# TUMFTM/RadarGNN

Hardware: AMD Instinct MI355X
Metric: radar frames/sec (graph-build + GNN fwd) (higher is better)
Workload: dtype f32 (dense layers: fp32 operands split into 2 f16 terms after an exact power-of-two pre-scale, 3 f16 MFMA products per fp32 product, fp32 accumulate -- more accurate than fp32 MFMA against float64, tests/test_gpu_f16x2.py; RGNN_NO_F16X2=1 selects 3 bf16 terms / 6 products, RGNN_LINEAR_FP32=1 v_mfma_; 1 GPU; C2: per GPU 64 RadarScenes-shaped frames x 3000 pts, radius graph r=1.0, node feats [rcs,velocity_vector,time_index,degree], edge feats [relative_position], 4-layer MPNNConv [224,224,128,64] + emb MLPs + both heads, train-mode BatchNorm, max aggr; frames_per_gpu=64, points_per_gpu=192000, edges_per_gpu=799078, ranks_in_process_group=1

## Files before the change

### include/rgnn.h

```cpp
#ifndef RGNN_H
#define RGNN_H

#include <stdint.h>

#ifdef __cplusplus
extern "C" {
#endif

typedef void* rgnn_stream_t;

#define RGNN_OK 0
#define RGNN_ERR_INVALID_ARGUMENT (-1)
#define RGNN_ERR_LAUNCH (-2)
#define RGNN_ERR_UNSUPPORTED (-3)

#define RGNN_STATUS_KNN_TOO_FEW_POINTS 1
#define RGNN_STATUS_DOT_PRODUCT 2
#define RGNN_STATUS_TIME_INDEX_OVERFLOW 4
#define RGNN_STATUS_EDGE_COUNT_CHANGED 8
#define RGNN_STATUS_NOT_SYMMETRIC 16
#define RGNN_STATUS_SPLITK_TIMEOUT 32
#define RGNN_STATUS_GT_OBJECT_TOO_LARGE 64
#define RGNN_STATUS_GT_DEGENERATE_OBJECT 128
#define RGNN_STATUS_PREPROCESS_BAD_ROW 256
// ... 214 lines not shown
                                const float* in_bound, float* out_bound, rgnn_stream_t stream);
int rgnn_batchnorm_segments_from_panels(const float* stats_a, const int32_t* panel_start_a, const float* stats_b,
                                        const int32_t* panel_start_b, const int64_t* seg_ptr, int64_t n_seg, int32_t n,
                                        const float* gamma, const float* beta, float* running_mean, float* running_var,
                                        int64_t* num_batches_tracked, float momentum, float eps, double* seg_sums, float* table,
                                        const float* in_bound, float* out_bound, rgnn_stream_t stream);
int rgnn_pad_list_by_segment(const int32_t* list, const int64_t* count, const int64_t* seg_ptr, int64_t n_seg, int32_t* out_list,
                             int64_t* out_count, int32_t* tile_segment, int32_t* stat_panel_start, rgnn_stream_t stream);
int rgnn_pad_list_pair_by_segment(const int32_t* list_a, const int64_t* count_a, const int32_t* list_b, const int64_t* count_b,
                                  const int64_t* seg_ptr, int64_t n_seg, int32_t* out_list_a, int64_t* out_count_a,
                                  int32_t* tile_segment_a, int32_t* stat_panel_start_a, int32_t* out_list_b, int64_t* out_count_b,
                                  int32_t* tile_segment_b, int32_t* stat_panel_start_b, rgnn_stream_t stream);
int rgnn_scale_shift_act_segments(const float* x, int64_t ldx, const float* table, const int64_t* seg_ptr, int64_t n_seg,
                                  int64_t m, int32_t n, int32_t relu, float* y, int64_t ldy, rgnn_stream_t stream);
int rgnn_column_stats(const float* x, int64_t ldx, int64_t m, int32_t n, float* col_stats ,
                      rgnn_stream_t stream);
int rgnn_scale_shift_act(const float* x, int64_t ldx, const float* scale_shift, int64_t m, int32_t n, int32_t relu,
                         float* y, int64_t ldy, rgnn_stream_t stream);

#define RGNN_AGGR_MAX 0
#define RGNN_AGGR_MEAN 1
#define RGNN_AGGR_ADD 2
int rgnn_mpnn_aggregate(const float* P, int64_t ldp, const float* p_bias, const float* Q, int64_t ldq,
                        const float* We , int64_t ldwe, const float* edge_attr_sorted,
                        int32_t de, const int32_t* rowptr_t, const int32_t* src_sorted,
                        const int32_t* node_order ,
                        const int32_t* chunk_start , int32_t n_chunks, int64_t n,
                        int32_t d, int32_t aggr, float* out, int64_t ldo, rgnn_stream_t stream);

#define RGNN_MPNN_SKIP_EMPTY_ROWS 1
int rgnn_mpnn_aggregate_flags(const float* P, int64_t ldp, const float* p_bias, const float* Q, int64_t ldq,
                              const float* We, int64_t ldwe, const float* edge_attr_sorted, int32_t de,
                              const int32_t* rowptr_t, const int32_t* src_sorted, const int32_t* node_order,
                              const int32_t* chunk_start, int32_t n_chunks, int64_t n, int32_t d, int32_t aggr, float* out,
                              int64_t ldo, int32_t flags, rgnn_stream_t stream);
int rgnn_mpnn_aggregate_absmax(const float* P, int64_t ldp, const float* p_bias, const float* Q, int64_t ldq,
                               const float* We, int64_t ldwe, const float* edge_attr_sorted, int32_t de,
                               const int32_t* rowptr_t, const int32_t* src_sorted, const int32_t* node_order,
                               const int32_t* chunk_start, int32_t n_chunks, int64_t n, int32_t d, int32_t aggr, float* out,
                               int64_t ldo, int32_t flags, float* out_absmax, rgnn_stream_t stream);
int rgnn_mpnn_aggregate_max_arg(const float* p_bias, const float* Q, int64_t ldq, const float* We, int64_t ldwe,
                                const float* edge_attr_sorted, int32_t de, const int32_t* rowptr_t, const int32_t* src_sorted,
                                const int32_t* node_order, const int32_t* chunk_start, int32_t n_chunks, int64_t n, int32_t d,
                                float* out, int64_t ldo, uint16_t* arg_out, int32_t flags, int32_t* arg_written ,
                                rgnn_stream_t stream);
int rgnn_mpnn_aggregate_max_arg_absmax(const float* p_bias, const float* Q, int64_t ldq, const float* We, int64_t ldwe,
                                       const float* edge_attr_sorted, int32_t de, const int32_t* rowptr_t, const int32_t* src_sorted,
                                       const int32_t* node_order, const int32_t* chunk_start, int32_t n_chunks, int64_t n, int32_t d,
                                       float* out, int64_t ldo, uint16_t* arg_out, int32_t flags, int32_t* arg_written ,
                                       float* out_absmax, rgnn_stream_t stream);

int64_t rgnn_mpnn_win_plan_ints(int64_t n, int64_t n_edges);
void rgnn_mpnn_win_plan_counters(int64_t n, int64_t n_edges, int64_t* leftover_word , int64_t* windows_word );
int rgnn_mpnn_win_plan(const int32_t* rowptr_t, const int32_t* src_sorted, const int32_t* node_order, int64_t n, int64_t n_edges,
                       int32_t* plan, rgnn_stream_t stream);
int rgnn_mpnn_aggregate_win(const float* p_bias, const float* Q, int64_t ldq, const float* We, int64_t ldwe,
                            const float* edge_attr_sorted, int32_t de, const int32_t* rowptr_t, const int32_t* src_sorted,
                            const int32_t* node_order, int32_t* plan, int64_t n, int64_t n_edges, int32_t d, float* out, int64_t ldo,
                            int32_t flags, float* out_absmax, rgnn_stream_t stream);
int64_t rgnn_mpnn_win_wplanes_bytes(int32_t d);
int rgnn_mpnn_win_wplanes(const float* We, int64_t ldwe, int32_t de, int32_t d, const float* p_bias, void* planes, rgnn_stream_t stream);
int rgnn_mpnn_aggregate_win_planes(const float* p_bias, const float* Q, int64_t ldq, const float* We, int64_t ldwe,
                                   const float* edge_attr_sorted, int32_t de, const int32_t* rowptr_t, const int32_t* src_sorted,
                                   const int32_t* node_order, int32_t* plan, int64_t n, int64_t n_edges, int32_t d, float* out,
                                   int64_t ldo, int32_t flags, float* out_absmax, const void* wplanes, rgnn_stream_t stream);

int rgnn_empty_targets(const int32_t* rowptr_t, const int32_t* node_order, int64_t n, int32_t* flags_tmp,
                       int32_t* pos_tmp, void* scan_tmp, int32_t* list, int64_t* count,
                       int32_t* slot_of_node ,
                       rgnn_stream_t stream);

int rgnn_split_targets(const int32_t* rowptr_t, const int32_t* node_order, int64_t n, int32_t* flags_tmp, int32_t* pos_tmp,
                       void* scan_tmp, int32_t* list, int64_t* count, int32_t* slot_of_node, int32_t* list_nonempty,
                       int64_t* count_nonempty, rgnn_stream_t stream);

int rgnn_split_targets_by_node(const int32_t* rowptr_t, const int32_t* rank, int64_t n, int32_t* flags_tmp, int32_t* pos_tmp,
                               void* scan_tmp, int32_t* list, int64_t* count, int32_t* slot_of_node,
                               int32_t* list_nonempty, int64_t* count_nonempty, rgnn_stream_t stream);

int32_t rgnn_mpnn_num_chunks(int64_t n, int64_t n_edges);
int32_t rgnn_mpnn_work_units(int64_t n, int64_t n_edges);
int32_t rgnn_mpnn_target_weight(int64_t n, int64_t n_edges);
int rgnn_mpnn_partition(const int32_t* rowptr_t, int64_t n, int64_t n_edges, int32_t* chunk_start, rgnn_stream_t stream);

int rgnn_mpnn_edge_hidden(const float* P, int64_t ldp, const float* p_bias, const float* Q, int64_t ldq,
                          const float* We, int64_t ldwe, const float* edge_attr_sorted, int32_t de,
                          const int32_t* rowptr_t, const int32_t* src_sorted, const int32_t* node_order,
                          const int32_t* chunk_start, int32_t n_chunks, int64_t n, int32_t d, int32_t relu, float* hidden,
                          int64_t ldh, rgnn_stream_t stream);
int rgnn_segment_reduce(const float* rows, int64_t ldr, const int32_t* rowptr_t, const int32_t* node_order, int64_t n,
                        int32_t d, int32_t aggr, float* out, int64_t ldo, rgnn_stream_t stream);

int rgnn_gather_rows_f32(const float* in, int64_t ldi, const int32_t* perm, int64_t n_rows, int32_t width, float* out,
                         int64_t ldo, rgnn_stream_t stream);

int rgnn_softmax_rows(const float* x, int64_t ldx, int64_t m, int32_t n, float* y, int64_t ldy, rgnn_stream_t stream);

int rgnn_collate_rows(const void* src, int64_t ld_src, int32_t width, const int64_t* seg_src_row, const int64_t* seg_dst_ptr,
                      int32_t n_seg, int64_t n_rows, void* out, int64_t ld_out, int64_t* batch_out, rgnn_stream_t stream);
int rgnn_collate_edges(const int64_t* src_edge_index, int64_t ld_src, const int64_t* seg_src_edge,
                       const int64_t* seg_dst_eptr, const int64_t* seg_node_shift, int32_t n_seg, int64_t n_edges,
                       int64_t* out, int64_t ld_out, rgnn_stream_t stream);

int rgnn_stage_frames(int64_t n_frames, const void* const* addr, const int64_t* n_points, void* block, int64_t block_bytes);

int rgnn_decode_predictions(const float* class_prob, int64_t ldp, int32_t n_classes, const float* boxes, int64_t ldb,
// ... 139 lines not shown
```

### radargnn_amd/_lib.py

```python
from __future__ import annotations

import ctypes as C
import os

import torch

_HERE = os.path.dirname(os.path.abspath(__file__))
LIB_PATH = os.environ.get("RGNN_LIB") or os.path.join(_HERE, "librgnn.so")

c_i32, c_i64, c_f32, c_f64, c_vp = C.c_int32, C.c_int64, C.c_float, C.c_double, C.c_void_p


class RgnnGrid(C.Structure):
    _fields_ = [("X", c_vp), ("dim", c_i32), ("n", c_i64), ("frame_ptr", c_vp), ("n_frames", c_i64),
                ("ws", c_vp), ("ws_bytes", c_i64)]


class RgnnLinearArgs(C.Structure):
    _fields_ = [("A1", c_vp), ("lda1", c_i64), ("k1", c_i32),
                ("A2", c_vp), ("lda2", c_i64), ("k2", c_i32),
                ("W1", c_vp), ("W2", c_vp), ("ldw", c_i64), ("w_split", c_i32),
                ("bias1", c_vp), ("bias2", c_vp),
                ("residual", c_vp), ("ldr", c_i64),
                ("out", c_vp), ("ldo", c_i64),
# ... 46 lines not shown
                            c_vp, c_vp]),
    "rgnn_csr_by_target_symmetric_own": (c_i32, [c_vp, c_vp, c_i64, c_i64, c_vp, c_vp, c_vp, c_vp, c_vp, c_vp, c_vp]),
    "rgnn_edge_features": (c_i32, [c_vp, c_vp, c_vp, c_i64, C.POINTER(c_i32), c_i32, c_i32, c_vp, c_i32, c_vp, c_vp]),
    "rgnn_edge_features_reversed": (c_i32, [c_vp, c_vp, c_vp, c_i64, c_vp, c_i64, C.POINTER(c_i32), c_i32, c_i32, c_vp, c_i32, c_vp, c_vp]),
    "rgnn_node_features": (c_i32, [c_vp, c_vp, c_vp, c_vp, c_vp, c_i64, C.POINTER(c_i32), c_i32, c_vp, c_i32, c_vp]),
    "rgnn_node_features_time_index": (c_i32, [c_vp, c_vp, c_vp, c_vp, c_vp, c_i64, c_vp, c_i64, C.POINTER(c_i32), c_i32, c_vp, c_i32,
                                              c_vp, c_vp, c_vp]),
    "rgnn_split_by_degree_frames": (c_i32, [c_vp, c_vp, c_i64, c_vp, c_vp, c_vp, c_vp, c_vp, c_vp, c_vp]),
    "rgnn_radius_counts": (c_i32, [c_vp, c_i64, c_vp, c_i32, c_vp, c_vp]),
    "rgnn_time_index": (c_i32, [c_vp, c_vp, c_i64, c_vp, c_vp, c_vp]),
    "rgnn_time_index_ws_bytes": (c_i64, [c_i64]),
    "rgnn_time_index_ws": (c_i32, [c_vp, c_vp, c_i64, c_i64, c_vp, c_vp, c_vp, c_i64, c_vp]),
    "rgnn_linear_stat_panels": (c_i64, [c_i64]),
    "rgnn_linear_fwd": (c_i32, [C.POINTER(RgnnLinearArgs), c_vp]),
    "rgnn_linear_fwd_fuses_a1_affine": (c_i32, [C.POINTER(RgnnLinearArgs)]),
    "rgnn_linear_fwd_plan": (None, [C.POINTER(RgnnLinearArgs), C.POINTER(c_i32 * 8)]),
    "rgnn_linear_planes_kp": (c_i32, [c_i32]),
    "rgnn_linear_fwd_path": (c_i32, [C.POINTER(RgnnLinearArgs)]),
    "rgnn_linear_planes_f16_bytes": (c_i64, [c_i32, c_i32]),
    "rgnn_linear_split_weights_f16": (c_i32, [c_vp, c_vp, c_i64, c_i32, c_i32, c_i32, c_vp, c_vp]),
    "rgnn_linear_splitk_ws_bytes": (c_i64, []),
    "rgnn_linear_split_weights": (c_i32, [c_vp, c_vp, c_i64, c_i32, c_i32, c_i32, c_vp, c_vp]),
    "rgnn_tiny_mlp2": (c_i32, [c_vp, c_i64, c_i32, c_vp, c_i64, c_vp, c_i64, c_vp, c_i32, c_i32, c_vp, c_i64, c_vp, c_i32, c_i32, c_vp,
                       c_i64, c_vp]),
    "rgnn_batchnorm_finalize": (c_i32, [c_vp, c_i64, c_i64, c_i32, c_vp, c_vp, c_vp, c_vp, c_vp, c_i32, c_f32, c_f32,
                                        c_vp, c_vp]),
    "rgnn_batchnorm_finalize_parts": (c_i32, [c_vp, c_i64, c_vp, c_vp, c_i64, c_vp, c_i64, c_i32, c_vp, c_vp, c_vp, c_vp, c_vp, c_i32,
                                              c_f32, c_f32, c_vp, c_vp]),
    "rgnn_batchnorm_finalize_bound": (c_i32, [c_vp, c_i64, c_vp, c_vp, c_i64, c_vp, c_i64, c_i32, c_vp, c_vp, c_vp, c_vp, c_vp, c_i32,
                                              c_f32, c_f32, c_vp, c_vp, c_vp, c_vp]),
    "rgnn_batchnorm_segments": (c_i32, [c_vp, c_i64, c_vp, c_i64, c_i32, c_vp, c_vp, c_vp, c_vp, c_vp, c_f32, c_f32, c_vp, c_vp,
                                        c_vp, c_vp, c_vp]),
    "rgnn_batchnorm_act_segments": (c_i32, [c_vp, c_i64, c_vp, c_i64, c_i32, c_vp, c_vp, c_vp, c_vp, c_vp, c_f32, c_f32, c_i32, c_vp,
                                            c_vp, c_vp, c_i64, c_vp, c_vp, c_vp]),
    "rgnn_batchnorm_segments_from_panels": (c_i32, [c_vp, c_vp, c_vp, c_vp, c_vp, c_i64, c_i32, c_vp, c_vp, c_vp, c_vp, c_vp, c_f32,
                                                    c_f32, c_vp, c_vp, c_vp, c_vp, c_vp]),
    "rgnn_pad_list_by_segment": (c_i32, [c_vp, c_vp, c_vp, c_i64, c_vp, c_vp, c_vp, c_vp, c_vp]),
    "rgnn_pad_list_pair_by_segment": (c_i32, [c_vp, c_vp, c_vp, c_vp, c_vp, c_i64, c_vp, c_vp, c_vp, c_vp, c_vp, c_vp, c_vp, c_vp, c_vp]),
    "rgnn_scale_shift_act_segments": (c_i32, [c_vp, c_i64, c_vp, c_vp, c_i64, c_i64, c_i32, c_i32, c_vp, c_i64, c_vp]),
    "rgnn_column_stats": (c_i32, [c_vp, c_i64, c_i64, c_i32, c_vp, c_vp]),
    "rgnn_scale_shift_act": (c_i32, [c_vp, c_i64, c_vp, c_i64, c_i32, c_i32, c_vp, c_i64, c_vp]),
    "rgnn_mpnn_aggregate": (c_i32, [c_vp, c_i64, c_vp, c_vp, c_i64, c_vp, c_i64, c_vp, c_i32, c_vp, c_vp, c_vp, c_vp, c_i32,
                                    c_i64, c_i32, c_i32, c_vp, c_i64, c_vp]),
    "rgnn_mpnn_aggregate_flags": (c_i32, [c_vp, c_i64, c_vp, c_vp, c_i64, c_vp, c_i64, c_vp, c_i32, c_vp, c_vp, c_vp, c_vp, c_i32,
                                          c_i64, c_i32, c_i32, c_vp, c_i64, c_i32, c_vp]),
    "rgnn_mpnn_aggregate_absmax": (c_i32, [c_vp, c_i64, c_vp, c_vp, c_i64, c_vp, c_i64, c_vp, c_i32, c_vp, c_vp, c_vp, c_vp, c_i32,
                                           c_i64, c_i32, c_i32, c_vp, c_i64, c_i32, c_vp, c_vp]),
    "rgnn_mpnn_aggregate_max_arg": (c_i32, [c_vp, c_vp, c_i64, c_vp, c_i64, c_vp, c_i32, c_vp, c_vp, c_vp, c_vp, c_i32, c_i64, c_i32,
                                             c_vp, c_i64, c_vp, c_i32, C.POINTER(c_i32), c_vp]),
    "rgnn_mpnn_aggregate_max_arg_absmax": (c_i32, [c_vp, c_vp, c_i64, c_vp, c_i64, c_vp, c_i32, c_vp, c_vp, c_vp, c_vp, c_i32, c_i64, c_i32,
                                                    c_vp, c_i64, c_vp, c_i32, C.POINTER(c_i32), c_vp, c_vp]),
    "rgnn_mpnn_win_plan_ints": (c_i64, [c_i64, c_i64]),
    "rgnn_mpnn_win_plan_counters": (None, [c_i64, c_i64, C.POINTER(c_i64), C.POINTER(c_i64)]),
    "rgnn_mpnn_win_plan": (c_i32, [c_vp, c_vp, c_vp, c_i64, c_i64, c_vp, c_vp]),
    "rgnn_mpnn_aggregate_win": (c_i32, [c_vp, c_vp, c_i64, c_vp, c_i64, c_vp, c_i32, c_vp, c_vp, c_vp, c_vp, c_i64, c_i64, c_i32, c_vp,
                                        c_i64, c_i32, c_vp, c_vp]),
    "rgnn_mpnn_win_wplanes_bytes": (c_i64, [c_i32]),
    "rgnn_mpnn_win_wplanes": (c_i32, [c_vp, c_i64, c_i32, c_i32, c_vp, c_vp, c_vp]),
    "rgnn_mpnn_aggregate_win_planes": (c_i32, [c_vp, c_vp, c_i64, c_vp, c_i64, c_vp, c_i32, c_vp, c_vp, c_vp, c_vp, c_i64, c_i64, c_i32, c_vp,
                                               c_i64, c_i32, c_vp, c_vp, c_vp]),
    "rgnn_empty_targets": (c_i32, [c_vp, c_vp, c_i64, c_vp, c_vp, c_vp, c_vp, c_vp, c_vp, c_vp]),
    "rgnn_split_targets": (c_i32, [c_vp, c_vp, c_i64, c_vp, c_vp, c_vp, c_vp, c_vp, c_vp, c_vp, c_vp, c_vp]),
    "rgnn_split_targets_by_node": (c_i32, [c_vp, c_vp, c_i64, c_vp, c_vp, c_vp, c_vp, c_vp, c_vp, c_vp, c_vp, c_vp]),
    "rgnn_mpnn_num_chunks": (c_i32, [c_i64, c_i64]),
    "rgnn_mpnn_work_units": (c_i32, [c_i64, c_i64]),
    "rgnn_mpnn_target_weight": (c_i32, [c_i64, c_i64]),
    "rgnn_mpnn_partition": (c_i32, [c_vp, c_i64, c_i64, c_vp, c_vp]),
    "rgnn_mpnn_edge_hidden": (c_i32, [c_vp, c_i64, c_vp, c_vp, c_i64, c_vp, c_i64, c_vp, c_i32, c_vp, c_vp, c_vp, c_vp, c_i32,
                                      c_i64, c_i32, c_i32, c_vp, c_i64, c_vp]),
    "rgnn_segment_reduce": (c_i32, [c_vp, c_i64, c_vp, c_vp, c_i64, c_i32, c_i32, c_vp, c_i64, c_vp]),
    "rgnn_gather_rows_f32": (c_i32, [c_vp, c_i64, c_vp, c_i64, c_i32, c_vp, c_i64, c_vp]),
    "rgnn_softmax_rows": (c_i32, [c_vp, c_i64, c_i64, c_i32, c_vp, c_i64, c_vp]),
    "rgnn_relu_bwd": (c_i32, [c_vp, c_vp, c_vp, c_i64, c_vp]),
    "rgnn_bn_bwd_stats": (c_i32, [c_vp, c_i64, c_vp, c_i64, c_vp, c_i64, c_i64, c_i32, c_vp, c_vp]),
    "rgnn_bn_bwd_apply": (c_i32, [c_vp, c_i64, c_vp, c_i64, c_vp, c_i64, c_vp, c_i64, c_i32, c_vp, c_i64, c_vp]),
    "rgnn_bn_bwd_stats_table": (c_i32, [c_vp, c_i64, c_vp, c_i64, c_vp, c_vp, c_i64, c_i64, c_i32, c_vp, c_vp]),
    "rgnn_bn_bwd_apply_table": (c_i32, [c_vp, c_i64, c_vp, c_i64, c_vp, c_vp, c_i64, c_vp, c_i64, c_i32, c_vp, c_i64, c_vp, c_vp]),
    "rgnn_bn_bwd_apply_absmax": (c_i32, [c_vp, c_i64, c_vp, c_i64, c_vp, c_i64, c_vp, c_i64, c_i32, c_vp, c_i64, c_vp, c_vp]),
    "rgnn_bn_bwd_coef": (c_i32, [c_vp, c_i64, c_vp, c_vp, c_vp, c_i64, c_i64, c_i32, c_vp, c_f32, c_i32, c_vp, c_vp, c_vp, c_vp]),
    "rgnn_mpnn_aggregate_bwd": (c_i32, [c_vp, c_i64, c_vp, c_i64, c_vp, c_i64, c_vp, c_i32, c_vp, c_vp, c_vp, c_i64, c_i32,
                                        c_i32, c_vp, c_vp, c_vp, c_vp, c_i64, c_vp, c_vp, c_vp, c_vp, c_i64, c_vp, c_vp, c_vp]),
    "rgnn_mpnn_max_bwd_supported": (c_i32, [c_i32, c_i32]),
    "rgnn_mpnn_max_bwd": (c_i32, [c_vp, c_i64, c_vp, c_i64, c_vp, c_i64, c_vp, c_i32, c_vp, c_vp, c_vp, c_vp, c_vp, c_i64, c_i32, c_vp,
                                   c_vp, c_vp, c_i64, c_vp, c_i32, c_vp, c_vp, c_i64, c_vp, c_vp, c_vp]),
    "rgnn_mpnn_max_bwd_absmax": (c_i32, [c_vp, c_i64, c_vp, c_i64, c_vp, c_i64, c_vp, c_i32, c_vp, c_vp, c_vp, c_vp, c_vp, c_i64, c_i32, c_vp,
                                          c_vp, c_vp, c_i64, c_vp, c_i32, c_vp, c_vp, c_i64, c_vp, c_vp, c_vp, c_vp]),
    "rgnn_mpnn_bwd_split": (c_i32, [c_i32]),
    "rgnn_segment_reduce_bwd": (c_i32, [c_vp, c_i64, c_vp, c_i64, c_vp, c_vp, c_i64, c_i32, c_i32, c_vp, c_i64, c_vp]),
    "rgnn_linear_wgrad_slabs": (c_i32, [c_i64, c_i32, c_i32]),
    "rgnn_linear_wgrad": (c_i32, [c_vp, c_i64, c_vp, c_i64, c_i32, c_vp, c_i64, c_i32, c_i64, c_i32, c_vp, c_vp, c_vp]),
    "rgnn_wgrad_slabs": (c_i32, [c_i64, c_i32, c_i32, c_i32, c_i32]),
    "rgnn_wgrad": (c_i32, [c_vp, c_i64, c_i32, c_vp, c_i64, c_i32, c_vp, c_i64, c_i32, c_i32, c_i64, c_vp, c_vp, c_vp, c_vp, c_vp]),
    "rgnn_wgrad_bounds": (c_i32, [c_vp, c_i64, c_i32, c_vp, c_i64, c_i32, c_vp, c_i64, c_i32, c_i32, c_i64, c_vp, c_vp, c_vp, c_vp, c_vp, c_vp,
                                   c_vp, c_vp]),
    "rgnn_mpnn_bwd_slots": (c_i64, [c_i64]),
    "rgnn_decode_predictions": (c_i32, [c_vp, c_i64, c_i32, c_vp, c_i64, c_i32, c_vp, c_vp, c_i64, c_i32, C.c_float, c_vp, c_i32,
                                        c_i32, c_i32, c_vp, c_vp, c_vp, c_vp, c_vp]),
    "rgnn_box_representations": (c_i32, [c_vp, c_i64, c_vp, c_vp, c_vp]),
    "rgnn_sort_scores_tmp_bytes": (c_i64, [c_i64]),
    "rgnn_sort_scores": (c_i32, [c_vp, c_i32, c_i64, c_vp, c_vp, c_vp]),
    "rgnn_nms_mask_words": (c_i64, [c_i64]),
    "rgnn_nms": (c_i32, [c_vp, c_i32, c_vp, c_i64, c_f64, c_vp, c_vp, c_vp, c_vp]),
    "rgnn_decode_ground_truth": (c_i32, [c_vp, c_i64, c_vp, c_i64, c_i32, c_vp, c_vp, c_i64, c_i32, c_i32, c_vp, c_vp, c_vp]),
    "rgnn_remove_duplicate_boxes": (c_i32, [c_vp, c_vp, c_i64, c_i64, c_vp, c_vp]),
    "rgnn_point_iou_tmp_bytes": (c_i64, [c_i64, c_i32, c_i64, c_i64]),
    "rgnn_point_iou": (c_i32, [c_vp, c_vp, c_i64, c_vp, c_vp, c_i64, c_i32, c_vp, c_vp, c_i64, c_i32, c_vp, c_i64, c_vp, c_vp, c_vp]),
# ... 55 lines not shown
```

### radargnn_amd/csrc/mpnn_tiles.hip

```cpp
#include "common.h"
#include <stdlib.h>
#include <type_traits>

namespace {

constexpr int MT_THREADS = 256;
constexpr int MT_WAVES = MT_THREADS / 64;
constexpr int MT_QUEUE_INTS = 8 * 16;

typedef float mt_f32x16 __attribute__((ext_vector_type(16)));
typedef __bf16 mt_bf16x8 __attribute__((ext_vector_type(8)));
typedef unsigned int mt_u32x4 __attribute__((ext_vector_type(4)));

__global__ __launch_bounds__(256) void k_tiles_zero_empty(const int32_t* __restrict__ rowptr, const int32_t* __restrict__ order,
                                                         int64_t n, int d, float* __restrict__ out, int64_t ldo) {
  const int lane = threadIdx.x & 63;
  const int64_t p = (int64_t)blockIdx.x * MT_WAVES + (threadIdx.x >> 6);
  if (p >= n || rowptr[p + 1] != rowptr[p]) return;
  const int64_t node = order ? order[p] : p;
  for (int c = lane; c < d; c += 64) out[node * ldo + c] = 0.f;
}

__device__ __forceinline__ void mt_split3(float x, unsigned& t1, unsigned& t2, unsigned& t3) {
  t1 = __float_as_uint(x) & 0xffff0000u;
// ... 262 lines not shown
#pragma unroll
          for (int i = 0; i < 16; i++) c[i] = *(const __attribute__((address_space(3))) float*)(uintptr_t)(unsigned)(aoff[t][i] + ST * WN_ROWBUF);
          c = __builtin_amdgcn_mfma_f32_32x32x16_bf16(__builtin_bit_cast(mt_bf16x8, a3[t]), __builtin_bit_cast(mt_bf16x8, byc), c, 0, 0, 0);
          c = __builtin_amdgcn_mfma_f32_32x32x16_bf16(__builtin_bit_cast(mt_bf16x8, a2[t]), __builtin_bit_cast(mt_bf16x8, bxc), c, 0, 0, 0);
          c = __builtin_amdgcn_mfma_f32_32x32x16_bf16(__builtin_bit_cast(mt_bf16x8, a1[t]), __builtin_bit_cast(mt_bf16x8, bxc), c, 0, 0, 0);
#pragma unroll
          for (int g = 0; g < WN_GPT; g++) {
            rn = __builtin_fmaxf(__builtin_fmaxf(rn, c[WN_PAD * g]), c[WN_PAD * g + 1]);
            if (WN_PAD == 4) rn = __builtin_fmaxf(__builtin_fmaxf(rn, c[WN_PAD * g + 2]), c[WN_PAD * g + 3]);
            if ((anyend >> (WN_GPT * t + g)) & 1u) {
              const int k = WN_GPT * t + g;
              const float v = rn + biasc;
              const unsigned long long mA = ((endA >> k) & 1u) ? 0xffffffffull : 0ull, mB = ((endB >> k) & 1u) ? 0xffffffff00000000ull : 0ull;
              const int soA = __builtin_amdgcn_readlane(tv, k) + ct * 128, soB = __builtin_amdgcn_readlane(tv, 32 + k) + ct * 128;
              if (!(p.abl & 4)) {
                const int off = (half ? soB : soA) + voffc;
                asm volatile("s_mov_b64 exec, %3\n\tbuffer_store_dword %0, %1, %2, 0 offen nt\n\ts_mov_b64 exec, -1"
                             : : "v"(v), "v"(off), "s"(ro_l), "s"(mA | mB) : "memory");
              }
              if (AMAX) amax = fmaxf(amax, fabsf(v));
              const unsigned long long m64 = mA | mB;
              asm volatile("v_cndmask_b32_e64 %0, %0, %1, %2" : "+v"(rn) : "v"(ninf_l), "s"(m64));
            }
          }
        }
      }
    };
    float amax_full = 0.f;
    for (int ct = 0; ct < p.n_ct; ct++) {
      const bool partial = AMAX && (ct + 1) * 32 > p.d;
      if (partial) { amax_full = amax; amax = 0.f; }
      if ((gp + ct) & 1) tile_pass(ct, std::integral_constant<int, 1>());
      else tile_pass(ct, std::integral_constant<int, 0>());
      if (partial) amax = fmaxf(amax_full, (ct * 32 + col < p.d) ? amax : 0.f);
    }
    if (p.n_ct < 2) {
      asm volatile("s_waitcnt vmcnt(0)" ::: "memory");
      __syncthreads();
    }
    gp = (gp + p.n_ct) & 1;
    win = nxt; up ^= 1; staged = staged_next;
  }
  if (AMAX) {
#pragma unroll
    for (int o = 32; o > 0; o >>= 1) amax = fmaxf(amax, __shfl_xor(amax, o, 64));
    if (lane == 0)
      atomicMax((unsigned int*)p.out_absmax + ((blockIdx.x * 4 + wave) & (RGNN_BOUND_SLOTS - 1)), __float_as_uint(amax));
  }
}

constexpr int WN_BIG = 64;

constexpr int WN_SEG = 512;
struct WinPlanLayout {
  int n_win, n_seg;
  int64_t off_assign, off_segcnt, off_segbase, off_wend, off_pdeg, off_wstart, off_left, off_leftcnt, off_queue, off_misc, off_tgt, off_eid, off_lrow, off_urow,
      off_wplanes, total_ints;
};
WinPlanLayout win_layout(int64_t n, int64_t n_edges) {
  WinPlanLayout L;
  L.n_seg = (int)((n + WN_SEG - 1) / WN_SEG);
  L.n_win = (int)((n_edges + 3 * n) / 256 + L.n_seg + 2);
  int64_t o = 16;
  auto take = [&](int64_t ints) { const int64_t at = o; o = (o + ints + 15) / 16 * 16; return at; };
  L.off_assign = take(n + 1); L.off_segcnt = take(L.n_seg + 1); L.off_segbase = take(L.n_seg + 2);
  L.off_wend = take(L.n_win + 1);
  L.off_pdeg = take(n + 1); L.off_wstart = take(L.n_win + 1); L.off_left = take(n + 1); L.off_leftcnt = take(4);
  L.off_queue = take(MT_QUEUE_INTS); L.off_misc = take(16 * (int64_t)L.n_win);
  L.off_tgt = take(8 * WN_GPS * (int64_t)L.n_win); L.off_eid = take(512 * (int64_t)L.n_win); L.off_lrow = take(128 * (int64_t)L.n_win);
  L.off_urow = take(WN_UMAX * (int64_t)L.n_win); L.off_wplanes = take(16 * 64 * 32);
  L.total_ints = o;
  return L;
}

__global__ __launch_bounds__(256) void k_win_pdeg(const int32_t* __restrict__ rowptr, int64_t n, int32_t* __restrict__ pdeg,
                                                 int32_t* __restrict__ left, int32_t* __restrict__ leftcnt, int32_t* __restrict__ queue) {
  const int64_t p = (int64_t)blockIdx.x * blockDim.x + threadIdx.x;
  if (p < MT_QUEUE_INTS) queue[p] = 0;
  if (p > n) return;
  if (p == n) { pdeg[p] = 0; return; }
  const int d = rowptr[p + 1] - rowptr[p];
  const int pd = (d + WN_PAD - 1) & ~(WN_PAD - 1);
  if (pd > WN_BIG) left[atomicAdd(leftcnt, 1)] = (int32_t)p;
  pdeg[p] = (pd > WN_BIG) ? 0 : pd;
}
__global__ __launch_bounds__(64) void k_win_greedy(const int32_t* __restrict__ pdeg, int64_t n, int32_t* __restrict__ assign,
                                                  int32_t* __restrict__ segcnt) {
  __shared__ int spd[WN_SEG];
  __shared__ int sas[WN_SEG];
  const int seg = blockIdx.x, lane = threadIdx.x;
  const int64_t p0 = (int64_t)seg * WN_SEG;
  const int cnt = (int)min((int64_t)WN_SEG, n - p0);
  for (int i = lane; i < cnt; i += 64) spd[i] = pdeg[p0 + i];
  __syncthreads();
  {
    int fill = 0;
    int win = 0, any = 0;
    for (int ib = 0; ib < cnt; ib += 64) {
      const int mine_pd = (ib + lane < cnt) ? spd[ib + lane] : 0;
      int mine_as = -1;
      const int nb = min(64, cnt - ib);
      for (int j = 0; j < nb; j++) {
        const int pd = __builtin_amdgcn_readlane(mine_pd, j);
        if (pd == 0) continue;
        const unsigned long long fits = __ballot(lane < 8 && fill + pd <= 64);
        int b = 0;
        if (fits == 0) { win++; fill = 0; }
        else b = __builtin_ctzll(fits);
        const int off = __builtin_amdgcn_readlane(fill, b);
        if (lane == b) fill += pd;
        any = 1;
        if (lane == j) mine_as = (win << 16) | (b * 64 + off);
      }
      if (ib + lane < cnt) sas[ib + lane] = mine_as;
    }
    if (lane == 0) segcnt[seg] = any ? win + 1 : 0;
  }
  __syncthreads();
  for (int i = lane; i < cnt; i += 64) assign[p0 + i] = sas[i];
}
__global__ __launch_bounds__(1024) void k_win_segbase(const int32_t* __restrict__ segcnt, int n_seg, int32_t* __restrict__ segbase) {
  __shared__ int part[1024];
  const int t = threadIdx.x;
  const int per = (n_seg + 1023) / 1024;
  int sum = 0;
  for (int i = t * per; i < min(n_seg, (t + 1) * per); i++) sum += segcnt[i];
  part[t] = sum;
  __syncthreads();
  for (int o = 1; o < 1024; o <<= 1) {
    const int v = t >= o ? part[t - o] : 0;
    __syncthreads();
    part[t] += v;
    __syncthreads();
  }
  int run = part[t] - sum;
  for (int i = t * per; i < min(n_seg, (t + 1) * per); i++) { segbase[i] = run; run += segcnt[i]; }
  if (t == 1023) segbase[n_seg] = part[1023];
}
__global__ __launch_bounds__(256) void k_win_starts(const int32_t* __restrict__ assign, const int32_t* __restrict__ segbase, int64_t n, int n_seg,
                                                   int n_win, int32_t* __restrict__ wstart, int32_t* __restrict__ wend) {
  const int64_t p = (int64_t)blockIdx.x * blockDim.x + threadIdx.x;
  if (p >= n) return;
  const int a = assign[p];
  if (a < 0) return;
  const int seg = (int)(p / WN_SEG);
  const int w = segbase[seg] + (a >> 16);
  if (w >= n_win) return;
  if ((a & 0xffff) == 0) wstart[w] = (int32_t)p;
  atomicMax(&wend[w], (int32_t)p + 1);
}

__global__ __launch_bounds__(256) void k_win_pack(const int32_t* __restrict__ rowptr, const int32_t* __restrict__ src,
                                                 const int32_t* __restrict__ order, const int32_t* __restrict__ pdeg,
                                                 const int32_t* __restrict__ assign, const int32_t* __restrict__ segbase,
                                                 const int32_t* __restrict__ wstart, const int32_t* __restrict__ wend, int n_win,
                                                 int32_t* __restrict__ misc_out, int32_t* __restrict__ tgt_out,
                                                 int32_t* __restrict__ eid_out, uint8_t* __restrict__ lrow_out, int32_t* __restrict__ urow_out,
                                                 int32_t* __restrict__ left, int32_t* __restrict__ leftcnt) {
  __shared__ int s_src[4][512];
  __shared__ int s_key[4][1024];
  __shared__ int s_val[4][1024];
  __shared__ short s_assign[4][WN_TMAX];
  __shared__ int s_pos[4][WN_TMAX];
  __shared__ int s_pd[4][WN_TMAX];
  __shared__ int s_e0[4][WN_TMAX];
  __shared__ int s_misc[4][16];
  __shared__ int s_end[4][32];
  const int lane = threadIdx.x & 63, wv = threadIdx.x >> 6;
  const int w = blockIdx.x * 4 + wv;
  if (w >= n_win) return;
  const int p1 = wend[w], p0 = p1 > 0 ? wstart[w] : 0;
  int* ssrc = s_src[wv]; int* skey = s_key[wv]; int* sval = s_val[wv]; short* sas = s_assign[wv]; int* spos = s_pos[wv]; int* spd = s_pd[wv]; int* se0 = s_e0[wv]; int* misc = s_misc[wv]; int* send = s_end[wv];
  const int64_t wb = (int64_t)w * 512;
  if (p1 == 0) {
    if (lane < 16) misc_out[(int64_t)w * 16 + lane] = 0;
    return;
  }
  for (int i = lane; i < 512; i += 64) { ssrc[i] = -1; eid_out[wb + i] = 0; lrow_out[wb + i] = 0; }
  for (int i = lane; i < 1024; i += 64) skey[i] = -1;
  for (int i = lane; i < 8 * WN_GPS; i += 64) tgt_out[(int64_t)w * (8 * WN_GPS) + i] = 0;
  if (lane < 32) send[lane] = 0;
  if (lane == 0) misc[9] = 0;
  __builtin_amdgcn_s_waitcnt(0);
  __builtin_amdgcn_wave_barrier();
  for (int pb = p0; pb < p1; pb += 64) {
    const int p = pb + lane;
    const int a = p < p1 ? assign[p] : -1;
    const bool mine = a >= 0 && segbase[p / WN_SEG] + (a >> 16) == w;
    const unsigned long long m = __ballot(mine);
    const int base = misc[9];
    const int j = base + __popcll(m & ((1ull << lane) - 1ull));
    if (mine) {
      if (j < WN_TMAX) { spos[j] = p; spd[j] = pdeg[p]; se0[j] = rowptr[p]; sas[j] = (short)(a & 0xffff); }
      else left[atomicAdd(leftcnt, 1)] = p;
    }
    __builtin_amdgcn_s_waitcnt(0);
    __builtin_amdgcn_wave_barrier();
    if (lane == 0) misc[9] = min(base + __popcll(m), WN_TMAX);
    __builtin_amdgcn_s_waitcnt(0);
    __builtin_amdgcn_wave_barrier();
  }
  const int cnt = misc[9];
  if (lane < 8) misc[lane] = 0;
  __builtin_amdgcn_s_waitcnt(0);
  __builtin_amdgcn_wave_barrier();
  for (int i = lane; i < cnt; i += 64) atomicMax(&misc[sas[i] >> 6], (sas[i] & 63) + spd[i]);
  for (int i = lane; i < cnt; i += 64) {
    const int at = sas[i], p = spos[i], e0 = se0[i], pd = spd[i];
    const int d = rowptr[p + 1] - e0;
    for (int q = 0; q < pd; q++) {
      const int e = e0 + min(q, d - 1);
      eid_out[wb + at + q] = e;
      ssrc[at + q] = src[e];
    }
    const int gi = ((at & 63) + pd - WN_PAD) / WN_PAD, b = at >> 6;
    atomicOr(&send[b * 4 + gi / WN_GPT], 1 << (gi % WN_GPT));
    tgt_out[(int64_t)w * (8 * WN_GPS) + b * WN_GPS + gi] = order ? order[p] : p;
  }
  __builtin_amdgcn_s_waitcnt(0);
  __builtin_amdgcn_wave_barrier();
  if (lane == 0) misc[8] = 0;
  for (int i = lane; i < 512; i += 64) {
    const int s_ = ssrc[i];
    if (s_ < 0) continue;
    unsigned h = ((unsigned)s_ * 2654435761u) >> 22;
    for (;;) {
      const int prev = atomicCAS(&skey[h], -1, s_);
      if (prev == -1 || prev == s_) break;
      h = (h + 1) & 1023;
    }
  }
  __builtin_amdgcn_s_waitcnt(0);
  __builtin_amdgcn_wave_barrier();
  for (int i = lane; i < 1024; i += 64)
    if (skey[i] >= 0) sval[i] = atomicAdd(&misc[8], 1);
  __builtin_amdgcn_s_waitcnt(0);
  __builtin_amdgcn_wave_barrier();
  const int nU = misc[8];
  if (nU > WN_UMAX) {
    for (int i = lane; i < cnt; i += 64) left[atomicAdd(leftcnt, 1)] = spos[i];
    if (lane < 16) misc_out[(int64_t)w * 16 + lane] = 0;
    return;
  }
  for (int i = lane; i < 1024; i += 64)
    if (skey[i] >= 0) urow_out[(int64_t)w * WN_UMAX + sval[i]] = skey[i];
  for (int i = lane; i < 512; i += 64) {
// ... 45 lines not shown
#pragma unroll
        for (int k = 0; k < 8; k++) my_z[k] = k < de ? ea[(int64_t)el * de + k] : 0.f;
        const int nb = min(64, e1 - eb);
        for (int q = 0; q < nb; q += 8) {
          float v[8][2];
          int jj[8];
#pragma unroll
          for (int u = 0; u < 8; u++) {
            jj[u] = min(q + u, nb - 1);
            const int64_t r = (int64_t)__builtin_amdgcn_readlane(my_src, jj[u]) * ldq + cw + lane;
#pragma unroll
            for (int j = 0; j < 2; j++) v[u][j] = ok[j] ? Q[r + 64 * j] : 0.f;
          }
#pragma unroll
          for (int u = 0; u < 8; u++) {
            float z[8];
#pragma unroll
            for (int k = 0; k < 8; k++) z[k] = __builtin_bit_cast(float, __builtin_amdgcn_readlane(__builtin_bit_cast(int, my_z[k]), jj[u]));
#pragma unroll
            for (int j = 0; j < 2; j++) {
#pragma unroll
              for (int k = 0; k < 8; k++) v[u][j] = __builtin_fmaf(w[j][k], z[k], v[u][j]);
              m[j] = fmaxf(m[j], v[u][j]);
            }
          }
        }
      }
#pragma unroll
      for (int j = 0; j < 2; j++) {
        if (!ok[j]) continue;
        const int c = cw + 64 * j + lane;
        const float o = m[j] + (p_bias ? p_bias[c] : 0.f);
        out[node * ldo + c] = o;
        amax = fmaxf(amax, fabsf(o));
      }
    }
  }
  if (out_absmax != nullptr) {
#pragma unroll
    for (int o = 32; o > 0; o >>= 1) amax = fmaxf(amax, __shfl_xor(amax, o, 64));
    if (lane == 0 && amax > 0.f)
      atomicMax((unsigned int*)out_absmax + ((blockIdx.x * 4 + wv) & (RGNN_BOUND_SLOTS - 1)), __float_as_uint(amax));
  }
}

}

extern "C" int64_t rgnn_mpnn_win_plan_ints(int64_t n, int64_t n_edges) { return win_layout(n, n_edges).total_ints; }
extern "C" void rgnn_mpnn_win_plan_counters(int64_t n, int64_t n_edges, int64_t* leftover_word, int64_t* windows_word) {
  const WinPlanLayout L = win_layout(n, n_edges);
  *leftover_word = L.off_leftcnt;
  *windows_word = L.off_segbase + L.n_seg;
}

extern "C" int rgnn_mpnn_win_plan(const int32_t* rowptr_t, const int32_t* src_sorted, const int32_t* node_order, int64_t n, int64_t n_edges,
                                  int32_t* plan, rgnn_stream_t stream) {
  RGNN_CHECK_ARG(rowptr_t && plan && n >= 0 && n_edges >= 0, "bad arguments");
  RGNN_CHECK_ARG(n_edges == 0 || src_sorted, "null src_sorted");
  RGNN_CHECK_ARG((((uintptr_t)plan) & 15) == 0, "plan must be 16-byte aligned");
  if (n == 0) return RGNN_OK;
  const WinPlanLayout L = win_layout(n, n_edges);
  hipStream_t s = (hipStream_t)stream;
  hipMemsetAsync(plan + L.off_leftcnt, 0, 16, s);
  hipLaunchKernelGGL(k_win_pdeg, dim3(rgnn_blocks(n + 1 > MT_QUEUE_INTS ? n + 1 : MT_QUEUE_INTS, 256)), dim3(256), 0, s, rowptr_t, n, plan + L.off_pdeg,
                     plan + L.off_left, plan + L.off_leftcnt, plan + L.off_queue);
  hipMemsetAsync(plan + L.off_wend, 0, 4 * (size_t)(L.n_win + 1), s);
  hipLaunchKernelGGL(k_win_greedy, dim3(L.n_seg), dim3(64), 0, s, (const int32_t*)(plan + L.off_pdeg), n, plan + L.off_assign, plan + L.off_segcnt);
  hipLaunchKernelGGL(k_win_segbase, dim3(1), dim3(1024), 0, s, (const int32_t*)(plan + L.off_segcnt), L.n_seg, plan + L.off_segbase);
  hipLaunchKernelGGL(k_win_starts, dim3(rgnn_blocks(n, 256)), dim3(256), 0, s, (const int32_t*)(plan + L.off_assign),
                     (const int32_t*)(plan + L.off_segbase), n, L.n_seg, L.n_win, plan + L.off_wstart, plan + L.off_wend);
  hipLaunchKernelGGL(k_win_pack, dim3(rgnn_blocks(L.n_win, 4)), dim3(256), 0, s, rowptr_t, src_sorted, node_order,
                     (const int32_t*)(plan + L.off_pdeg), (const int32_t*)(plan + L.off_assign), (const int32_t*)(plan + L.off_segbase),
                     (const int32_t*)(plan + L.off_wstart), (const int32_t*)(plan + L.off_wend), L.n_win, plan + L.off_misc,
                     plan + L.off_tgt, plan + L.off_eid, (uint8_t*)(plan + L.off_lrow),
                     plan + L.off_urow, plan + L.off_left, plan + L.off_leftcnt);
  RGNN_CHECK_LAUNCH();
  return RGNN_OK;
}

extern "C" int64_t rgnn_mpnn_win_wplanes_bytes(int32_t d) { return d < 1 ? -1 : (int64_t)((d + 31) / 32) * WN_BBUF; }

extern "C" int rgnn_mpnn_win_wplanes(const float* We, int64_t ldwe, int32_t de, int32_t d, const float* p_bias, void* planes,
                                     rgnn_stream_t stream) {
  RGNN_CHECK_ARG(planes && d >= 1 && de >= 0 && de <= 8 && (de == 0 || We) && (((uintptr_t)planes) & 15) == 0, "bad arguments");
  const int n_ct = (d + 31) / 32;
  hipLaunchKernelGGL(k_win_wplanes, dim3(rgnn_blocks(n_ct * 32, 256)), dim3(256), 0, (hipStream_t)stream, We, (int)ldwe, de, d, n_ct, p_bias,
                     (mt_u32x4*)planes);
  RGNN_CHECK_LAUNCH();
  return RGNN_OK;
}

static int aggregate_win(const float* p_bias, const float* Q, int64_t ldq, const float* We, int64_t ldwe,
                         const float* edge_attr_sorted, int32_t de, const int32_t* rowptr_t, const int32_t* src_sorted,
                         const int32_t* node_order, int32_t* plan, int64_t n, int64_t n_edges, int32_t d, float* out,
                         int64_t ldo, int32_t flags, float* out_absmax, const void* wplanes, rgnn_stream_t stream) {
  if (n == 0) return RGNN_OK;
  RGNN_CHECK_ARG(Q && rowptr_t && plan && out && d >= 1, "bad arguments");
  RGNN_CHECK_ARG((flags & ~RGNN_MPNN_SKIP_EMPTY_ROWS) == 0, "unknown flags");
  RGNN_CHECK_ARG(de == 0 || ((We || wplanes) && edge_attr_sorted), "edge attributes given without weights");
  RGNN_CHECK_ARG((((uintptr_t)wplanes) & 15) == 0, "operand image not 16-byte aligned");
  const int64_t q_bytes = ((n - 1) * ldq + d) * 4, o_bytes = ((n - 1) * ldo + d) * 4;
  if (de > 8 || d > 2048 || n >= ((int64_t)1 << 24) || ldq * 4 >= ((int64_t)1 << 24) || q_bytes >= ((int64_t)1 << 31) ||
      o_bytes >= ((int64_t)1 << 31) || (ldq % 4) != 0 || (((uintptr_t)Q) & 15) != 0 || win_layout(n, n_edges).total_ints * 4 >= ((int64_t)1 << 31)) {
    rgnn_set_error("rgnn_mpnn_aggregate_win: shape not covered (de %d, d %d, n %lld, ldq %lld)", de, d, (long long)n, (long long)ldq);
    return RGNN_ERR_UNSUPPORTED;
  }
  hipStream_t s = (hipStream_t)stream;
  if (!(flags & RGNN_MPNN_SKIP_EMPTY_ROWS))
    hipLaunchKernelGGL(k_tiles_zero_empty, dim3(rgnn_blocks(n, MT_WAVES)), dim3(256), 0, s, rowptr_t, node_order, n, d, out, ldo);
  if (n_edges > 0) {
    const WinPlanLayout L = win_layout(n, n_edges);
    WinParams p;
    p.p_bias = p_bias; p.Q = Q; p.ldq4 = (int)(ldq * 4); p.q_bytes = (int)q_bytes;
    p.wplanes = wplanes ? (const mt_u32x4*)wplanes : (const mt_u32x4*)(plan + L.off_wplanes); p.ea = edge_attr_sorted; p.de = de;
    p.ea_vec = (de == 8 && (((uintptr_t)edge_attr_sorted) & 15) == 0) ? 1 : 0;
    p.n_win = L.n_win; p.n_win_dev = plan + L.off_segbase + L.n_seg;
    p.plan = plan; p.plan_bytes = (int)(L.total_ints * 4);
    p.off_misc = (int)(L.off_misc * 4); p.off_eid = (int)(L.off_eid * 4); p.off_lrow = (int)(L.off_lrow * 4); p.off_urow = (int)(L.off_urow * 4); p.off_tgt = (int)(L.off_tgt * 4);
    p.queue = plan + L.off_queue;
    p.d = d; p.n_ct = (d + 31) / 32; p.out = out; p.ldo4 = (int)(ldo * 4); p.o_bytes = (int)o_bytes; p.out_absmax = out_absmax;
    p.abl = RGNN_ENV("RGNN_MPNN_WIN_ABL") ? atoi(RGNN_ENV("RGNN_MPNN_WIN_ABL")) : 0;
    if (!wplanes)
      hipLaunchKernelGGL(k_win_wplanes, dim3(rgnn_blocks(p.n_ct * 32, 256)), dim3(256), 0, s, We, (int)ldwe, de, d, p.n_ct, p_bias,
                         (mt_u32x4*)(plan + L.off_wplanes));
    const size_t lds = WN_LDS;
    static RgnnOncePerDevice attr_once;
    if (attr_once.first()) {
// ... 36 lines not shown
```

Before: 31890 frames/s.

## Fuse window-plan build into greedy kernel with last-block segment scan

```diff
diff --git a/include/rgnn.h b/include/rgnn.h
--- a/include/rgnn.h
+++ b/include/rgnn.h
@@ -290,6 +290,7 @@
 
 int64_t rgnn_mpnn_win_plan_ints(int64_t n, int64_t n_edges);
 void rgnn_mpnn_win_plan_counters(int64_t n, int64_t n_edges, int64_t* leftover_word , int64_t* windows_word );
+void rgnn_mpnn_win_plan_words(int64_t n, int64_t n_edges, int64_t* words );
 int rgnn_mpnn_win_plan(const int32_t* rowptr_t, const int32_t* src_sorted, const int32_t* node_order, int64_t n, int64_t n_edges,
                        int32_t* plan, rgnn_stream_t stream);
 int rgnn_mpnn_aggregate_win(const float* p_bias, const float* Q, int64_t ldq, const float* We, int64_t ldwe,
diff --git a/radargnn_amd/_lib.py b/radargnn_amd/_lib.py
--- a/radargnn_amd/_lib.py
+++ b/radargnn_amd/_lib.py
@@ -122,6 +122,7 @@
                                                     c_vp, c_i64, c_vp, c_i32, C.POINTER(c_i32), c_vp, c_vp]),
     "rgnn_mpnn_win_plan_ints": (c_i64, [c_i64, c_i64]),
     "rgnn_mpnn_win_plan_counters": (None, [c_i64, c_i64, C.POINTER(c_i64), C.POINTER(c_i64)]),
+    "rgnn_mpnn_win_plan_words": (None, [c_i64, c_i64, C.POINTER(c_i64)]),
     "rgnn_mpnn_win_plan": (c_i32, [c_vp, c_vp, c_vp, c_i64, c_i64, c_vp, c_vp]),
     "rgnn_mpnn_aggregate_win": (c_i32, [c_vp, c_vp, c_i64, c_vp, c_i64, c_vp, c_i32, c_vp, c_vp, c_vp, c_vp, c_i64, c_i64, c_i32, c_vp,
                                         c_i64, c_i32, c_vp, c_vp]),
diff --git a/radargnn_amd/csrc/mpnn_tiles.hip b/radargnn_amd/csrc/mpnn_tiles.hip
--- a/radargnn_amd/csrc/mpnn_tiles.hip
+++ b/radargnn_amd/csrc/mpnn_tiles.hip
@@ -338,9 +338,11 @@
 constexpr int WN_BIG = 64;
 
 constexpr int WN_SEG = 512;
+constexpr int WN_SEGWIN = WN_SEG / 8;
+constexpr int WN_ZERO_INTS = 16 + MT_QUEUE_INTS + 16;
 struct WinPlanLayout {
   int n_win, n_seg;
-  int64_t off_assign, off_segcnt, off_segbase, off_wend, off_pdeg, off_wstart, off_left, off_leftcnt, off_queue, off_misc, off_tgt, off_eid, off_lrow, off_urow,
+  int64_t off_assign, off_segcnt, off_segbase, off_wtab, off_left, off_leftcnt, off_queue, off_done, off_misc, off_tgt, off_eid, off_lrow, off_urow,
       off_wplanes, total_ints;
 };
 WinPlanLayout win_layout(int64_t n, int64_t n_edges) {
@@ -350,96 +352,104 @@
   int64_t o = 16;
   auto take = [&](int64_t ints) { const int64_t at = o; o = (o + ints + 15) / 16 * 16; return at; };
   L.off_assign = take(n + 1); L.off_segcnt = take(L.n_seg + 1); L.off_segbase = take(L.n_seg + 2);
-  L.off_wend = take(L.n_win + 1);
-  L.off_pdeg = take(n + 1); L.off_wstart = take(L.n_win + 1); L.off_left = take(n + 1); L.off_leftcnt = take(4);
-  L.off_queue = take(MT_QUEUE_INTS); L.off_misc = take(16 * (int64_t)L.n_win);
+  L.off_wtab = take(2 * WN_SEGWIN * (int64_t)L.n_seg);
+  L.off_left = take(n + 1);
+  L.off_leftcnt = take(16); L.off_queue = take(MT_QUEUE_INTS); L.off_done = take(16);
+  L.off_misc = take(16 * (int64_t)L.n_win);
   L.off_tgt = take(8 * WN_GPS * (int64_t)L.n_win); L.off_eid = take(512 * (int64_t)L.n_win); L.off_lrow = take(128 * (int64_t)L.n_win);
   L.off_urow = take(WN_UMAX * (int64_t)L.n_win); L.off_wplanes = take(16 * 64 * 32);
   L.total_ints = o;
   return L;
 }
 
-__global__ __launch_bounds__(256) void k_win_pdeg(const int32_t* __restrict__ rowptr, int64_t n, int32_t* __restrict__ pdeg,
-                                                 int32_t* __restrict__ left, int32_t* __restrict__ leftcnt, int32_t* __restrict__ queue) {
-  const int64_t p = (int64_t)blockIdx.x * blockDim.x + threadIdx.x;
-  if (p < MT_QUEUE_INTS) queue[p] = 0;
-  if (p > n) return;
-  if (p == n) { pdeg[p] = 0; return; }
-  const int d = rowptr[p + 1] - rowptr[p];
-  const int pd = (d + WN_PAD - 1) & ~(WN_PAD - 1);
-  if (pd > WN_BIG) left[atomicAdd(leftcnt, 1)] = (int32_t)p;
-  pdeg[p] = (pd > WN_BIG) ? 0 : pd;
-}
-__global__ __launch_bounds__(64) void k_win_greedy(const int32_t* __restrict__ pdeg, int64_t n, int32_t* __restrict__ assign,
-                                                  int32_t* __restrict__ segcnt) {
-  __shared__ int spd[WN_SEG];
+__device__ __forceinline__ int wn_padded(int d) { return (d + WN_PAD - 1) & ~(WN_PAD - 1); }
+
+__global__ __launch_bounds__(64) void k_win_greedy(const int32_t* __restrict__ rowptr, int64_t n, int n_seg, int32_t* __restrict__ assign,
+                                                  int32_t* segcnt, int32_t* __restrict__ segbase, int32_t* __restrict__ wtab,
+                                                  int32_t* __restrict__ left, int32_t* __restrict__ leftcnt, int32_t* __restrict__ done) {
+  __shared__ int srp[WN_SEG + 1];
   __shared__ int sas[WN_SEG];
+  __shared__ int swr[2 * WN_SEGWIN];
+  __shared__ int s_ticket;
   const int seg = blockIdx.x, lane = threadIdx.x;
   const int64_t p0 = (int64_t)seg * WN_SEG;
   const int cnt = (int)min((int64_t)WN_SEG, n - p0);
-  for (int i = lane; i < cnt; i += 64) spd[i] = pdeg[p0 + i];
+  for (int i = lane; i <= cnt; i += 64) srp[i] = rowptr[p0 + i];
   __syncthreads();
+  int n_made;
   {
-    int fill = 0;
+    unsigned long long fill8 = 0;
     int win = 0, any = 0;
     for (int ib = 0; ib < cnt; ib += 64) {
-      const int mine_pd = (ib + lane < cnt) ? spd[ib + lane] : 0;
+      int mine_pd = (ib + lane < cnt) ? wn_padded(srp[ib + lane + 1] - srp[ib + lane]) : 0;
+      const bool big = mine_pd > WN_BIG;
+      const unsigned long long bigs = __ballot(big);
+      if (bigs != 0) {
+        int base = 0;
+        if (lane == 0) base = atomicAdd(leftcnt, __popcll(bigs));
+        base = __builtin_amdgcn_readfirstlane(base);
+        if (big) left[base + __popcll(bigs & ((1ull << lane) - 1ull))] = (int32_t)(p0 + ib + lane);
+      }
+      if (big) mine_pd = 0;
       int mine_as = -1;
       const int nb = min(64, cnt - ib);
       for (int j = 0; j < nb; j++) {
         const int pd = __builtin_amdgcn_readlane(mine_pd, j);
         if (pd == 0) continue;
-        const unsigned long long fits = __ballot(lane < 8 && fill + pd <= 64);
-        int b = 0;
-        if (fits == 0) { win++; fill = 0; }
-        else b = __builtin_ctzll(fits);
-        const int off = __builtin_amdgcn_readlane(fill, b);
-        if (lane == b) fill += pd;
+        const unsigned k = (unsigned)(pd + 63) * 0x01010101u;
+        const unsigned long long full = (fill8 + (((unsigned long long)k << 32) | k)) & 0x8080808080808080ull;
+        int at = 0;
+        if (full == 0x8080808080808080ull) { win++; fill8 = (unsigned long long)pd; }
+        else {
+          const int sh = __builtin_ctzll(full ^ 0x8080808080808080ull) - 7;
+          at = (sh << 3) + (int)((fill8 >> sh) & 0xff);
+          fill8 += (unsigned long long)pd << sh;
+        }
         any = 1;
-        if (lane == j) mine_as = (win << 16) | (b * 64 + off);
+        if (lane == j) mine_as = (win << 16) | at;
       }
       if (ib + lane < cnt) sas[ib + lane] = mine_as;
-    }
-    if (lane == 0) segcnt[seg] = any ? win + 1 : 0;
+      const int w = mine_as >> 16;
+      const unsigned long long placed = __ballot(mine_as >= 0);
+      const unsigned long long later = lane < 63 ? placed & ~((2ull << lane) - 1ull) : 0ull;
+      const int w_next = __shfl(w, later ? __builtin_ctzll(later) : lane, 64);
+      if (mine_as >= 0 && w < WN_SEGWIN) {
+        if ((mine_as & 0xffff) == 0) swr[2 * w] = (int)(p0 + ib + lane);
+        if (later == 0 || w_next != w) swr[2 * w + 1] = (int)(p0 + ib + lane) + 1;
+      }
+    }
+    n_made = any ? win + 1 : 0;
   }
   __syncthreads();
   for (int i = lane; i < cnt; i += 64) assign[p0 + i] = sas[i];
-}
-__global__ __launch_bounds__(1024) void k_win_segbase(const int32_t* __restrict__ segcnt, int n_seg, int32_t* __restrict__ segbase) {
-  __shared__ int part[1024];
-  const int t = threadIdx.x;
-  const int per = (n_seg + 1023) / 1024;
-  int sum = 0;
-  for (int i = t * per; i < min(n_seg, (t + 1) * per); i++) sum += segcnt[i];
-  part[t] = sum;
+  for (int i = lane; i < 2 * min(n_made, WN_SEGWIN); i += 64) wtab[(int64_t)seg * (2 * WN_SEGWIN) + i] = swr[i];
+  if (lane == 0) __hip_atomic_store(&segcnt[seg], n_made, __ATOMIC_RELAXED, __HIP_MEMORY_SCOPE_AGENT);
+  __threadfence();
   __syncthreads();
-  for (int o = 1; o < 1024; o <<= 1) {
-    const int v = t >= o ? part[t - o] : 0;
-    __syncthreads();
-    part[t] += v;
-    __syncthreads();
-  }
-  int run = part[t] - sum;
-  for (int i = t * per; i < min(n_seg, (t + 1) * per); i++) { segbase[i] = run; run += segcnt[i]; }
-  if (t == 1023) segbase[n_seg] = part[1023];
-}
-__global__ __launch_bounds__(256) void k_win_starts(const int32_t* __restrict__ assign, const int32_t* __restrict__ segbase, int64_t n, int n_seg,
-                                                   int n_win, int32_t* __restrict__ wstart, int32_t* __restrict__ wend) {
-  const int64_t p = (int64_t)blockIdx.x * blockDim.x + threadIdx.x;
-  if (p >= n) return;
-  const int a = assign[p];
-  if (a < 0) return;
-  const int seg = (int)(p / WN_SEG);
-  const int w = segbase[seg] + (a >> 16);
-  if (w >= n_win) return;
-  if ((a & 0xffff) == 0) wstart[w] = (int32_t)p;
-  atomicMax(&wend[w], (int32_t)p + 1);
+  if (lane == 0) s_ticket = atomicAdd(done, 1);
+  __syncthreads();
+  if (s_ticket != n_seg - 1) return;
+  __threadfence();
+  int run = 0;
+  for (int sb = 0; sb < n_seg; sb += 64) {
+    const int i = sb + lane;
+    const int c = i < n_seg ? __hip_atomic_load(&segcnt[i], __ATOMIC_RELAXED, __HIP_MEMORY_SCOPE_AGENT) : 0;
+    int incl = c;
+#pragma unroll
+    for (int o = 1; o < 64; o <<= 1) {
+      const int v = __shfl_up(incl, o, 64);
+      if (lane >= o) incl += v;
+    }
+    if (i < n_seg) segbase[i] = run + incl - c;
+    run += __shfl(incl, 63, 64);
+  }
+  if (lane == 0) segbase[n_seg] = run;
 }
 
 __global__ __launch_bounds__(256) void k_win_pack(const int32_t* __restrict__ rowptr, const int32_t* __restrict__ src,
-                                                 const int32_t* __restrict__ order, const int32_t* __restrict__ pdeg,
-                                                 const int32_t* __restrict__ assign, const int32_t* __restrict__ segbase,
-                                                 const int32_t* __restrict__ wstart, const int32_t* __restrict__ wend, int n_win,
+                                                 const int32_t* __restrict__ order, const int32_t* __restrict__ assign,
+                                                 const int32_t* __restrict__ segbase, const int32_t* __restrict__ wtab, int n_seg,
+                                                 int n_win,
                                                  int32_t* __restrict__ misc_out, int32_t* __restrict__ tgt_out,
                                                  int32_t* __restrict__ eid_out, uint8_t* __restrict__ lrow_out, int32_t* __restrict__ urow_out,
                                                  int32_t* __restrict__ left, int32_t* __restrict__ leftcnt) {
@@ -454,14 +464,19 @@
   __shared__ int s_end[4][32];
   const int lane = threadIdx.x & 63, wv = threadIdx.x >> 6;
   const int w = blockIdx.x * 4 + wv;
-  if (w >= n_win) return;
-  const int p1 = wend[w], p0 = p1 > 0 ? wstart[w] : 0;
+  if (w >= n_win || w >= segbase[n_seg]) return;
+  int seg = 0;
+  for (int hi = n_seg - 1; seg < hi;) {
+    const int mid = (seg + hi) >> 1;
+    if (segbase[mid + 1] > w) hi = mid;
+    else seg = mid + 1;
+  }
+  const int local = w - segbase[seg];
+  if (local < 0 || local >= WN_SEGWIN) return;
+  const int32_t* range = wtab + ((int64_t)seg * WN_SEGWIN + local) * 2;
+  const int p0 = range[0], p1 = range[1];
   int* ssrc = s_src[wv]; int* skey = s_key[wv]; int* sval = s_val[wv]; short* sas = s_assign[wv]; int* spos = s_pos[wv]; int* spd = s_pd[wv]; int* se0 = s_e0[wv]; int* misc = s_misc[wv]; int* send = s_end[wv];
   const int64_t wb = (int64_t)w * 512;
-  if (p1 == 0) {
-    if (lane < 16) misc_out[(int64_t)w * 16 + lane] = 0;
-    return;
-  }
   for (int i = lane; i < 512; i += 64) { ssrc[i] = -1; eid_out[wb + i] = 0; lrow_out[wb + i] = 0; }
   for (int i = lane; i < 1024; i += 64) skey[i] = -1;
   for (int i = lane; i < 8 * WN_GPS; i += 64) tgt_out[(int64_t)w * (8 * WN_GPS) + i] = 0;
@@ -472,12 +487,12 @@
   for (int pb = p0; pb < p1; pb += 64) {
     const int p = pb + lane;
     const int a = p < p1 ? assign[p] : -1;
-    const bool mine = a >= 0 && segbase[p / WN_SEG] + (a >> 16) == w;
+    const bool mine = a >= 0 && (a >> 16) == local;
     const unsigned long long m = __ballot(mine);
     const int base = misc[9];
     const int j = base + __popcll(m & ((1ull << lane) - 1ull));
     if (mine) {
-      if (j < WN_TMAX) { spos[j] = p; spd[j] = pdeg[p]; se0[j] = rowptr[p]; sas[j] = (short)(a & 0xffff); }
+      if (j < WN_TMAX) { spos[j] = p; se0[j] = rowptr[p]; spd[j] = wn_padded(rowptr[p + 1] - se0[j]); sas[j] = (short)(a & 0xffff); }
       else left[atomicAdd(leftcnt, 1)] = p;
     }
     __builtin_amdgcn_s_waitcnt(0);
@@ -629,6 +644,11 @@
   *leftover_word = L.off_leftcnt;
   *windows_word = L.off_segbase + L.n_seg;
 }
+extern "C" void rgnn_mpnn_win_plan_words(int64_t n, int64_t n_edges, int64_t* words) {
+  const WinPlanLayout L = win_layout(n, n_edges);
+  words[0] = L.off_misc; words[1] = L.off_tgt; words[2] = L.off_eid; words[3] = L.off_lrow; words[4] = L.off_urow;
+  words[5] = L.off_left; words[6] = L.off_leftcnt; words[7] = L.off_segbase + L.n_seg;
+}
 
 extern "C" int rgnn_mpnn_win_plan(const int32_t* rowptr_t, const int32_t* src_sorted, const int32_t* node_order, int64_t n, int64_t n_edges,
                                   int32_t* plan, rgnn_stream_t stream) {
@@ -638,18 +658,13 @@
   if (n == 0) return RGNN_OK;
   const WinPlanLayout L = win_layout(n, n_edges);
   hipStream_t s = (hipStream_t)stream;
-  hipMemsetAsync(plan + L.off_leftcnt, 0, 16, s);
-  hipLaunchKernelGGL(k_win_pdeg, dim3(rgnn_blocks(n + 1 > MT_QUEUE_INTS ? n + 1 : MT_QUEUE_INTS, 256)), dim3(256), 0, s, rowptr_t, n, plan + L.off_pdeg,
-                     plan + L.off_left, plan + L.off_leftcnt, plan + L.off_queue);
-  hipMemsetAsync(plan + L.off_wend, 0, 4 * (size_t)(L.n_win + 1), s);
-  hipLaunchKernelGGL(k_win_greedy, dim3(L.n_seg), dim3(64), 0, s, (const int32_t*)(plan + L.off_pdeg), n, plan + L.off_assign, plan + L.off_segcnt);
-  hipLaunchKernelGGL(k_win_segbase, dim3(1), dim3(1024), 0, s, (const int32_t*)(plan + L.off_segcnt), L.n_seg, plan + L.off_segbase);
-  hipLaunchKernelGGL(k_win_starts, dim3(rgnn_blocks(n, 256)), dim3(256), 0, s, (const int32_t*)(plan + L.off_assign),
-                     (const int32_t*)(plan + L.off_segbase), n, L.n_seg, L.n_win, plan + L.off_wstart, plan + L.off_wend);
+  static_assert(WN_ZERO_INTS == 16 + MT_QUEUE_INTS + 16, "leftcnt, queue and done are zeroed by one fill");
+  hipMemsetAsync(plan + L.off_leftcnt, 0, 4 * (size_t)WN_ZERO_INTS, s);
+  hipLaunchKernelGGL(k_win_greedy, dim3(L.n_seg), dim3(64), 0, s, rowptr_t, n, L.n_seg, plan + L.off_assign, plan + L.off_segcnt,
+                     plan + L.off_segbase, plan + L.off_wtab, plan + L.off_left, plan + L.off_leftcnt, plan + L.off_done);
   hipLaunchKernelGGL(k_win_pack, dim3(rgnn_blocks(L.n_win, 4)), dim3(256), 0, s, rowptr_t, src_sorted, node_order,
-                     (const int32_t*)(plan + L.off_pdeg), (const int32_t*)(plan + L.off_assign), (const int32_t*)(plan + L.off_segbase),
-                     (const int32_t*)(plan + L.off_wstart), (const int32_t*)(plan + L.off_wend), L.n_win, plan + L.off_misc,
-                     plan + L.off_tgt, plan + L.off_eid, (uint8_t*)(plan + L.off_lrow),
+                     (const int32_t*)(plan + L.off_assign), (const int32_t*)(plan + L.off_segbase), (const int32_t*)(plan + L.off_wtab),
+                     L.n_seg, L.n_win, plan + L.off_misc, plan + L.off_tgt, plan + L.off_eid, (uint8_t*)(plan + L.off_lrow),
                      plan + L.off_urow, plan + L.off_left, plan + L.off_leftcnt);
   RGNN_CHECK_LAUNCH();
   return RGNN_OK;
```

Result: no change. 31940 frames/s (median of 3 runs) (+0.2%).
